# microscopic-image-analysis/DiffPointRasterisation.jl

Measured on AMD Instinct MI355X. Metric: M points/s fwd+bwd, 10M pts→256³ grid; HBM GB/s vs roofline, higher is better.
Workload: dtype f32

## Files before the change

diffpointrasterisation.jl_amd/csrc/dpr_tiled.hip:

```cpp
#include <hip/hip_runtime.h>

#include <cstring>
#include <mutex>
#include <set>
#include <type_traits>
#include <utility>

#include "dpr_tiled_impl.h"

namespace dpr {

template <int NO>
__device__ __forceinline__ int primary_tile(const int (&ref0)[NO], const TileGeom<NO>& tg) {
    int t = 0, stride = 1;
    bool in = true;
#pragma unroll
    for (int d = 0; d < NO; ++d) {
        const int r = ref0[d] < 0 ? 0 : ref0[d];
        int c = r / TileDims<NO>::T[d];
        if (d == NO - 1) {
            c -= tg.tz0;
            in = (unsigned)c < (unsigned)tg.nt[d];
        }
        t += c * stride;
// ... 422 lines not shown
                it.part_nparts = part | (k << 16);
                items[atomicAdd(&bstart[bucket], 1u)] = it;
            }
            if (k > 1) {
                slab_run += k;
                split_list[atomicAdd(&s_nsplit, 1u)] = (uint32_t)i;
            }
            run += c;
        }
    }
    if (threadIdx.x == 1023) tile_start[NT] = wbase + incl;
    __syncthreads();
    if (threadIdx.x == 0) *n_split = s_nsplit;
}

constexpr int kScanTiles = 32, kScanGroups = 1024 / kScanTiles;
__global__ __launch_bounds__(1024) void k_colscan(uint32_t* __restrict__ counts, int nblk, int NT,
                                                  uint32_t* __restrict__ totals,
                                                  uint32_t* __restrict__ zero_word = nullptr) {
    if (zero_word && blockIdx.x == 0 && threadIdx.x < 2) zero_word[threadIdx.x] = 0u;
    constexpr int kRowBatch = 16;
    __shared__ uint32_t part[kScanGroups][kScanTiles];
    const int j = threadIdx.x % kScanTiles, g = threadIdx.x / kScanTiles;
    const int tile = blockIdx.x * kScanTiles + j;
    const int rows = (nblk + kScanGroups - 1) / kScanGroups;
    const int r0 = g * rows, r1 = (r0 + rows < nblk) ? r0 + rows : nblk;
    const bool one = rows <= kRowBatch;
    const bool live = tile < NT;
    uint32_t v[kRowBatch];
    uint32_t s = 0;
    for (int rb = r0; rb < r1; rb += kRowBatch) {
#pragma unroll
        for (int k = 0; k < kRowBatch; ++k)
            v[k] = (live && rb + k < r1) ? counts[(size_t)(rb + k) * NT + tile] : 0u;
#pragma unroll
        for (int k = 0; k < kRowBatch; ++k) s += v[k];
    }
    part[g][j] = s;
    __syncthreads();
    uint32_t base = 0, total = 0;
#pragma unroll
    for (int k = 0; k < kScanGroups; ++k) {
        const uint32_t pv = part[k][j];
        if (k < g) base += pv;
        total += pv;
    }
    if (!live) return;
    for (int rb = r0; rb < r1; rb += kRowBatch) {
        if (!one) {
#pragma unroll
            for (int k = 0; k < kRowBatch; ++k)
                v[k] = (rb + k < r1) ? counts[(size_t)(rb + k) * NT + tile] : 0u;
        }
#pragma unroll
        for (int k = 0; k < kRowBatch; ++k) {
            if (rb + k < r1) counts[(size_t)(rb + k) * NT + tile] = base;
            base += v[k];
        }
    }
    if (g == 0) totals[tile] = total;
}

__global__ __launch_bounds__(1024) void k_tilescan(TileScanArgs ts) {
    tilescan_body(ts.totals, ts.NT, ts.cap, ts.tile_start, ts.items, ts.n_items, ts.tile_parts,
                  ts.tile_slab, ts.split_list, ts.n_split, ts.hdr, ts.hdr_out, ts.rot,
                  ts.rot_words, ts.trans, ts.trans_words, ts.nonzero_bins, ts.nblk);
}

}
#include "dpr_coarse.h"
namespace dpr {

template <typename T, int NI, int NO, bool HAS_PW, bool WANT_IDX>
__global__ __launch_bounds__(kBinThreads) void k_scatter(
    GridDesc<NO> gd, TileGeom<NO> tg, int64_t P, int64_t chunk, const T* __restrict__ points,
    const T* __restrict__ pw, const T* __restrict__ rot, const T* __restrict__ trans, int64_t b,
    const uint32_t* __restrict__ prefix, const uint32_t* __restrict__ tile_start,
    Rec4<T>* __restrict__ rec, uint32_t* __restrict__ rec_idx, uint32_t* __restrict__ slot_of,
    T* __restrict__ ds_dpoints, T* __restrict__ ds_dpw, int zero_dropped,
    uint32_t* __restrict__ maxpw) {
    extern __shared__ uint32_t cursor[];
    const unsigned slice = xcd_slice(blockIdx.x, gridDim.x);
    const uint32_t* row = prefix + (size_t)slice * tg.NT;
    for (int i = threadIdx.x; i < tg.NT; i += kBinThreads) cursor[i] = tile_start[i] + row[i];
    __syncthreads();
    const Pose<T, NI, NO> ps = load_pose<T, NI, NO>(rot, trans, nullptr, b);
    const int64_t lo = (int64_t)slice * chunk;
    const int64_t hi = (lo + chunk < P) ? lo + chunk : P;
    if (lo >= hi) return;
    uint32_t wkey = 0;
    int64_t p = lo + threadIdx.x;
    T nxt[NI], nxt_w = T(1);
    {
        const int64_t pl = p < hi ? p : hi - 1;
        load_point<T, NI>(points, pl, nxt);
        if (HAS_PW) nxt_w = pw[pl];
    }
#pragma unroll
    for (int j = 0; j < NI; ++j) pin_value(nxt[j]);
    if (HAS_PW) pin_value(nxt_w);
    drain_vmem();
    while (p < hi) {
        T pt[NI];
#pragma unroll
        for (int j = 0; j < NI; ++j) pt[j] = nxt[j];
        const T w = nxt_w;
        const int64_t pc = p;
        p += kBinThreads;
        {
            const int64_t pl = p < hi ? p : hi - 1;
            load_point<T, NI>(points, pl, nxt);
            if (HAS_PW) nxt_w = pw[pl];
        }
        int ref0[NO];
        T dlo[NO];
        bool valid = ref_and_deltas<T, NI, NO>(pt, ps, gd, ref0, dlo);
        const int tl = valid ? primary_tile<NO>(ref0, tg) : -1;
        valid = tl >= 0;
        uint32_t pos = (uint32_t)P;
        if (valid) pos = atomicAdd(&cursor[tl], 1u);
        if (HAS_PW && valid) wkey = wrange_merge(wkey, abs_key(w));
        Rec4<T> r;
#pragma unroll
        for (int j = 0; j < 3; ++j) r.v[j] = (j < NI) ? pt[(j < NI) ? j : 0] : T(0);
        r.v[3] = HAS_PW ? w : idx_to_slot((uint32_t)pc, T(0));
        rec[pos] = r;
        if (HAS_PW && WANT_IDX) rec_idx[pos] = (uint32_t)pc;
        if (WANT_IDX) slot_of[pc] = pos;
        if (zero_dropped && !valid) {
#pragma unroll
            for (int j = 0; j < NI; ++j) ds_dpoints[pc * NI + j] = T(0);
            if (ds_dpw) ds_dpw[pc] = T(0);
        }
    }
    if (HAS_PW) publish_max_abs(maxpw, wkey);
}

template <typename T, int NI, int NO, bool HAS_PW, int S, bool GROUP, bool W3, bool RUNS>
__device__ __forceinline__ void scatter_wc_body(
    const GridDesc<NO>& gd, const TileGeom<NO>& tg, int64_t P, int64_t chunk, const T* __restrict__ points,
    const T* __restrict__ pw, const T* __restrict__ rot, const T* __restrict__ trans, int64_t b0,
    int nb, const uint32_t* __restrict__ prefix, const uint32_t* __restrict__ tile_start,
    RecT<T, W3>* __restrict__ rec, uint32_t* __restrict__ slot_of, uint16_t* __restrict__ run_lp,
    T* __restrict__ ds_dpoints, T* __restrict__ ds_dpw, int zero_dropped, uint32_t* __restrict__ maxpw,
    int fused_scan, const TileScanArgs& ts) {
    const unsigned n_slices = fused_scan ? gridDim.x - 1u : gridDim.x;
    if (fused_scan && blockIdx.x == n_slices) {
        tilescan_body(ts.totals, ts.NT, ts.cap, ts.tile_start, ts.items, ts.n_items, ts.tile_parts,
                      ts.tile_slab, ts.split_list, ts.n_split, ts.hdr, ts.hdr_out, ts.rot,
                      ts.rot_words, ts.trans, ts.trans_words, ts.nonzero_bins, ts.nblk);
        return;
    }
    static_assert(!(W3 && HAS_PW), "compact records carry no point weight");
    static_assert(!RUNS || (!GROUP && !W3 && S <= 65536), "the sorted map: one pose, 4-word records, uint16 owners");
    constexpr int PPT = S / kWcThreads;
    uint32_t wkey = 0;
    if (!GROUP) nb = 1;
    const int NT = tg.NT, NTe = NT * nb;
    const uint32_t Pe = (uint32_t)(P * nb);
    extern __shared__ uint32_t dyn[];
    uint32_t* cursor = dyn;
    uint32_t* lhist = dyn + NTe;
    __shared__ RecT<T, W3> recs[S];
    __shared__ uint32_t dest[S];
    __shared__ uint16_t lpos[RUNS ? S : 1];
    uint32_t* const wsum = dest;
    static_assert(S >= kWcThreads / kWave, "wave sums fit");
    const unsigned slice = xcd_slice(blockIdx.x, n_slices);
    const uint32_t* row = prefix + (size_t)slice * NTe;
    constexpr int kMaxBpt = 4096 / kWcThreads;
    const int lane = threadIdx.x & (kWave - 1), wave = threadIdx.x / kWave;
    if (fused_scan) {
        const int bpe = (NTe + kWcThreads - 1) / kWcThreads;
        const int e0 = threadIdx.x * bpe;
        uint32_t c[kMaxBpt], rw[kMaxBpt], sum = 0;
#pragma unroll
        for (int q = 0; q < kMaxBpt; ++q) {
            const int i = e0 + q;
            const bool in = q < bpe && i < NTe;
            c[q] = in ? ts.totals[i] : 0u;
            rw[q] = in ? row[i] : 0u;
            sum += c[q];
        }
        uint32_t incl = sum;
#pragma unroll
        for (int o = 1; o < kWave; o <<= 1) {
            const uint32_t v = __shfl_up(incl, o, kWave);
            if (lane >= o) incl += v;
        }
        if (lane == kWave - 1) wsum[wave] = incl;
        __syncthreads();
        uint32_t run = incl - sum;
        for (int wv = 0; wv < wave; ++wv) run += wsum[wv];
#pragma unroll
        for (int q = 0; q < kMaxBpt; ++q) {
            const int i = e0 + q;
            if (q < bpe && i < NTe) cursor[i] = run + rw[q];
            run += c[q];
        }
    } else {
        for (int i = threadIdx.x; i < NTe; i += kWcThreads) cursor[i] = tile_start[i] + row[i];
    }
    for (int i = threadIdx.x; i < NT; i += kWcThreads) lhist[i] = 0;
    __syncthreads();
    const int64_t lo = (int64_t)slice * chunk;
    const int64_t hi = (lo + chunk < P) ? lo + chunk : P;
    const int bpt = (NT + kWcThreads - 1) / kWcThreads;
    const int bin0 = threadIdx.x * bpt;
    if (lo >= hi) return;
    constexpr bool kPrefetch = !GROUP;
    auto load_sub = [&](int64_t sbase, T (&dp)[PPT][NI], T (&dw)[PPT]) {
        const int64_t left = hi - sbase;
        const uint32_t n = left >= S ? (uint32_t)S : (left > 0 ? (uint32_t)left : 0u);
        const T* const pb = points + (n ? sbase : hi - 1) * NI;
        const T* const wb = HAS_PW ? pw + (n ? sbase : hi - 1) : nullptr;
#pragma unroll
        for (int k = 0; k < PPT; ++k) {
            const uint32_t lp = threadIdx.x + (uint32_t)k * kWcThreads;
            const uint32_t ll = n ? (lp < n ? lp : n - 1) : 0u;
            load_point<T, NI>(pb, (int64_t)ll, dp[k]);
            dw[k] = HAS_PW ? wb[ll] : T(1);
        }
    };
    T nxt_pt[kPrefetch ? PPT : 1][NI], nxt_w[kPrefetch ? PPT : 1];
    if constexpr (kPrefetch) load_sub(lo, nxt_pt, nxt_w);
    for (int64_t base = lo; base < hi; base += S) {
        const uint32_t nloc = (uint32_t)((hi - base < S) ? hi - base : S);
        T pt[PPT][NI], w[PPT];
        if constexpr (kPrefetch) {
#pragma unroll
            for (int k = 0; k < PPT; ++k) {
#pragma unroll
                for (int j = 0; j < NI; ++j) pt[k][j] = nxt_pt[k][j];
                w[k] = nxt_w[k];
            }
            load_sub(base + S, nxt_pt, nxt_w);
        } else {
            load_sub(base, pt, w);
        }
        for (int jp = 0; jp < (GROUP ? nb : 1); ++jp) {
            const Pose<T, NI, NO> ps = load_pose<T, NI, NO>(rot, trans, nullptr, b0 + jp);
            uint32_t* cur = cursor + jp * NT;
            uint32_t* const slot_b = slot_of ? slot_of + (size_t)jp * P + base : (uint32_t*)nullptr;
            int tile[PPT];
            uint32_t lrank[PPT];
#pragma unroll
            for (int k = 0; k < PPT; ++k) {
                const uint32_t lp = threadIdx.x + (uint32_t)k * kWcThreads;
                int ref0[NO];
                T dlo[NO];
                bool valid = ref_and_deltas<T, NI, NO>(pt[k], ps, gd, ref0, dlo) && lp < nloc;
                tile[k] = valid ? primary_tile<NO>(ref0, tg) : -1;
                valid = tile[k] >= 0;
                lrank[k] = 0;
                if (valid) lrank[k] = atomicAdd(&lhist[tile[k]], 1u);
                if (HAS_PW && valid) wkey = wrange_merge(wkey, abs_key(w[k]));
            }
            lds_barrier();
            uint32_t cnt_sum = 0;
            uint32_t cnt[kMaxBpt];
#pragma unroll
            for (int q = 0; q < kMaxBpt; ++q) {
                const int i = bin0 + q;
                cnt[q] = (q < bpt && i < NT) ? lhist[i] : 0u;
                cnt_sum += cnt[q];
            }
            uint32_t incl = cnt_sum;
#pragma unroll
            for (int o = 1; o < kWave; o <<= 1) {
                const uint32_t v = __shfl_up(incl, o, kWave);
                if (lane >= o) incl += v;
            }
            if (lane == kWave - 1) wsum[wave] = incl;
            lds_barrier();
            uint32_t run = incl - cnt_sum;
            for (int wv = 0; wv < wave; ++wv) run += wsum[wv];
            uint32_t n_valid = 0;
#pragma unroll
            for (int wv = 0; wv < kWcThreads / kWave; ++wv) n_valid += wsum[wv];
#pragma unroll
            for (int q = 0; q < kMaxBpt; ++q) {
                const int i = bin0 + q;
                if (q < bpt && i < NT) lhist[i] = run;
                run += cnt[q];
            }
            lds_barrier();
#pragma unroll
            for (int k = 0; k < PPT; ++k) {
                const uint32_t lp = threadIdx.x + (uint32_t)k * kWcThreads;
                if (tile[k] >= 0) {
                    const uint32_t sidx = lhist[tile[k]] + lrank[k];
                    const uint32_t d = cur[tile[k]] + lrank[k];
                    RecT<T, W3> r;
#pragma unroll
                    for (int j = 0; j < 3; ++j) r.v[j] = (j < NI) ? pt[k][(j < NI) ? j : 0] : T(0);
                    if constexpr (!W3) r.v[3] = HAS_PW ? w[k] : idx_to_slot((uint32_t)base + lp, T(0));
                    recs[sidx] = r;
                    dest[sidx] = d;
                    if constexpr (RUNS) lpos[sidx] = (uint16_t)lp;
                    else if (slot_b) __builtin_nontemporal_store(d, &slot_b[lp]);
                } else if (lp < nloc) {
                    if (!RUNS && slot_b) __builtin_nontemporal_store(Pe, &slot_b[lp]);
                    if (zero_dropped) {
                        T* const dp_b = ds_dpoints + base * NI;
#pragma unroll
                        for (int j = 0; j < NI; ++j) dp_b[lp * NI + j] = T(0);
                        if (ds_dpw) (ds_dpw + base)[lp] = T(0);
                    }
                }
            }
            lds_barrier();
            if constexpr (RUNS) {
                uint16_t* const lp_b = run_lp + base;
                for (uint32_t i = threadIdx.x; i < nloc; i += kWcThreads) {
                    const bool owned = i < n_valid;
                    const uint32_t d = dest[i];
                    if (owned) {
                        rec[d] = recs[i];
                        __builtin_nontemporal_store(lpos[i], &lp_b[i]);
                    }
                    __builtin_nontemporal_store(owned ? d : kRunEnd, &slot_b[i]);
                }
            } else {
                for (uint32_t i = threadIdx.x; i < n_valid; i += kWcThreads) rec[dest[i]] = recs[i];
            }
#pragma unroll
            for (int q = 0; q < kMaxBpt; ++q) {
                const int i = bin0 + q;
                if (q < bpt && i < NT) {
                    cur[i] += cnt[q];
                    lhist[i] = 0;
                }
            }
            lds_barrier();
        }
    }
    if (HAS_PW) publish_max_abs(maxpw, wkey);
}
template <typename T, int NI, int NO, bool HAS_PW, int S, bool GROUP, bool W3>
__global__ __launch_bounds__(kWcThreads) void k_scatter_wc(
    GridDesc<NO> gd, TileGeom<NO> tg, int64_t P, int64_t chunk, const T* __restrict__ points,
    const T* __restrict__ pw, const T* __restrict__ rot, const T* __restrict__ trans, int64_t b0,
    int nb, const uint32_t* __restrict__ prefix, const uint32_t* __restrict__ tile_start,
    RecT<T, W3>* __restrict__ rec, uint32_t* __restrict__ slot_of, T* __restrict__ ds_dpoints,
    T* __restrict__ ds_dpw, int zero_dropped, uint32_t* __restrict__ maxpw, int fused_scan,
    TileScanArgs ts) {
    scatter_wc_body<T, NI, NO, HAS_PW, S, GROUP, W3, false>(gd, tg, P, chunk, points, pw, rot, trans, b0, nb, prefix,
                                                            tile_start, rec, slot_of, nullptr, ds_dpoints, ds_dpw,
                                                            zero_dropped, maxpw, fused_scan, ts);
}
template <typename T, int NI, int NO, bool HAS_PW, int S>
__global__ __launch_bounds__(kWcThreads) void k_scatter_wc_runs(
    GridDesc<NO> gd, TileGeom<NO> tg, int64_t P, int64_t chunk, const T* __restrict__ points,
    const T* __restrict__ pw, const T* __restrict__ rot, const T* __restrict__ trans, int64_t b0,
    const uint32_t* __restrict__ prefix, const uint32_t* __restrict__ tile_start, Rec4<T>* __restrict__ rec,
    uint32_t* __restrict__ run_slot, uint16_t* __restrict__ run_lp, uint32_t* __restrict__ maxpw, int fused_scan,
    TileScanArgs ts) {
    scatter_wc_body<T, NI, NO, HAS_PW, S, false, false, true>(gd, tg, P, chunk, points, pw, rot, trans, b0, 1, prefix,
                                                              tile_start, rec, run_slot, run_lp, nullptr, nullptr, 0,
                                                              maxpw, fused_scan, ts);
}

struct LocalBinArgs {
    char* ws;
    size_t pose_stride;
    size_t off_rec, off_slot, off_desc, off_bdesc, off_ltot;
};
constexpr int kTouchCap = 1024;
template <typename T, int NI, int NO, bool HAS_PW, int S, bool W3, bool ONE, int TH, bool STAGE>
__global__ __launch_bounds__(TH, ((sizeof(T) == 4 && ONE) ? 8 : 4)) void k_bin_local(
    GridDesc<NO> gd, TileGeom<NO> tg, int64_t P, const T* __restrict__ points,
    const T* __restrict__ pw, const T* __restrict__ rot, const T* __restrict__ trans, int64_t b0,
    int nb, LocalBinArgs la, int want_slot, uint32_t spare_slot, T* __restrict__ ds_dpoints,
    T* __restrict__ ds_dpw, int zero_dropped) {
    static_assert(!(W3 && HAS_PW), "compact records carry no point weight");
    constexpr int PPT = S / TH;
    if (ONE) nb = 1;
    const int NT = tg.NT;
    extern __shared__ uint32_t lhist[];
    __shared__ RecT<T, W3> recs[STAGE ? S : 1];
    __shared__ uint16_t touched[kTouchCap];
    __shared__ uint32_t wsum[TH / kWave];
    __shared__ uint32_t s_ntouch, s_nvalid;
    for (int i = threadIdx.x; i < NT; i += TH) lhist[i] = 0;
    if (threadIdx.x == 0) s_ntouch = 0;
    const int64_t base = (int64_t)blockIdx.x * S;
    const uint32_t nloc = (uint32_t)((P - base < S) ? P - base : S);
    const T* const pts_blk = points + base * NI;
    const T* const pw_blk = HAS_PW ? pw + base : nullptr;
    T pt[PPT][NI], w[PPT];
#pragma unroll
    for (int k = 0; k < PPT; ++k) {
        const uint32_t lp = threadIdx.x + (uint32_t)k * TH;
        const uint32_t ll = lp < nloc ? lp : nloc - 1;
        if (nloc) {
            load_point<T, NI>(pts_blk, (int64_t)ll, pt[k]);
            w[k] = HAS_PW ? pw_blk[ll] : T(1);
        } else {
#pragma unroll
            for (int j = 0; j < NI; ++j) pt[k][j] = T(0);
            w[k] = T(1);
        }
    }
    if constexpr (HAS_PW) {
        uint32_t wkey = 0;
#pragma unroll
        for (int k = 0; k < PPT; ++k)
            if (threadIdx.x + (uint32_t)k * TH < nloc) wkey = wrange_merge(wkey, abs_key(w[k]));
        publish_max_abs((uint32_t*)(la.ws + la.off_ltot) + 2 * NT, wkey);
    }
    __syncthreads();
    const int lane = threadIdx.x & (kWave - 1), wave = threadIdx.x / kWave;
#pragma unroll 1
    for (int jp = 0; jp < nb; ++jp) {
        const Pose<T, NI, NO> ps = load_pose<T, NI, NO>(rot, trans, nullptr, b0 + jp);
        char* const wsp = la.ws + (size_t)jp * la.pose_stride;
        RecT<T, W3>* const rec_blk = (RecT<T, W3>*)(wsp + la.off_rec) + base;
        uint32_t* const slot_blk = want_slot ? (uint32_t*)(wsp + la.off_slot) + base : (uint32_t*)nullptr;
        RunDesc* const desc = (RunDesc*)(wsp + la.off_desc) + (size_t)blockIdx.x * S;
        uint32_t* const ltot = (uint32_t*)(wsp + la.off_ltot);
        int tile[PPT];
        uint32_t lrank[PPT];
        uint32_t left = 0;
#pragma unroll
        for (int k = 0; k < PPT; ++k) {
            const uint32_t lp = threadIdx.x + (uint32_t)k * TH;
            int ref0[NO];
            T dlo[NO];
            bool valid = ref_and_deltas<T, NI, NO>(pt[k], ps, gd, ref0, dlo) && lp < nloc;
            tile[k] = valid ? primary_tile<NO>(ref0, tg) : -1;
            valid = tile[k] >= 0;
            lrank[k] = 0;
            unsigned long long todo = __ballot(valid);
            int rounds = 0;
            while (todo && rounds < 8) {
                const int leader = __ffsll((long long)todo) - 1;
                const int t = __shfl(tile[k], leader, kWave);
                const unsigned long long same = __ballot(tile[k] == t) & todo;
                if (__popcll(same) < 4) break;
                uint32_t r0 = 0;
                if (lane == leader) {
                    r0 = atomicAdd(&lhist[t], (uint32_t)__popcll(same));
                    if (r0 == 0) {
                        const uint32_t pos = atomicAdd(&s_ntouch, 1u);
                        if (pos < (uint32_t)kTouchCap) touched[pos] = (uint16_t)t;
                    }
                }
                r0 = __shfl(r0, leader, kWave);
                if ((same >> lane) & 1ull) lrank[k] = r0 + (uint32_t)__popcll(same & ((1ull << lane) - 1ull));
                todo &= ~same;
                ++rounds;
            }
            if ((todo >> lane) & 1ull) left |= 1u << k;
        }
        if (__ballot(left != 0)) {
#pragma unroll
            for (int k = 0; k < PPT; ++k)
                if ((left >> k) & 1u) lrank[k] = atomicAdd(&lhist[tile[k]], 1u);
#pragma unroll
            for (int k = 0; k < PPT; ++k) {
                if (((left >> k) & 1u) && lrank[k] == 0) {
                    const uint32_t pos = atomicAdd(&s_ntouch, 1u);
                    if (pos < (uint32_t)kTouchCap) touched[pos] = (uint16_t)tile[k];
                }
            }
        }
        lds_barrier();
        const uint32_t n_t = s_ntouch;
        const bool listed = n_t <= (uint32_t)kTouchCap;
        if (listed) {
            if (wave == 0) {
                uint32_t carry = 0;
                for (uint32_t i0 = 0; i0 < n_t; i0 += kWave) {
                    const uint32_t i = i0 + lane;
// ... 1546 lines not shown
        }
    }
    const int lane = threadIdx.x & (kWave - 1), wave = threadIdx.x / kWave;
#pragma unroll
    for (int k = 0; k < NVAL; ++k) {
        const double v = (k < NVAL - 2) ? (double)vals[k < NVAL - 2 ? k : 0]
                                        : (k == NVAL - 2 ? bg_sum : sq_sum);
        const double s = wave_sum<double>(v);
        if (lane == 0) red[wave][k] = s;
    }
    __syncthreads();
    if (threadIdx.x < (rs.target ? NVAL : NVAL - 1)) {
        double s = 0.0;
#pragma unroll
        for (int w = 0; w < NW; ++w) s += red[w][threadIdx.x];
        partials[(size_t)threadIdx.x * max_items + blockIdx.x] = s;
    }
}

template <typename T> struct PoseReduceArgs {
    const double* partials;
    const WorkItem* items;
    const uint32_t* n_items;
    int max_items, NT, n_in, n_out;
    int64_t b0;
    T* ds_drotation;
    T* ds_dtranslation;
    T* ds_dbackground;
    T* ds_dout_weight;
    T* loss;
    BinHeader* hdr;
    int accumulate;
};
template <typename T>
__device__ __forceinline__ void pose_reduce_body(int k, uint32_t j, bool grouped,
                                                 const PoseReduceArgs<T>& a) {
    __shared__ double wsum[16];
    const int64_t b = a.b0 + j;
    double s = 0.0;
    const bool stale = a.hdr && a.hdr->verdict != 1u;
    if (a.hdr && k == 0 && j == 0 && threadIdx.x == 0) a.hdr->state = 0u;
    const int n = stale ? 0 : (int)*a.n_items;
    if (!grouped) {
        for (int t = threadIdx.x; t < n; t += 1024) s += a.partials[(size_t)k * a.max_items + t];
    } else {
        for (int t = threadIdx.x; t < n; t += 1024)
            if (a.items[t].tile / (uint32_t)a.NT == j) s += a.partials[(size_t)k * a.max_items + t];
    }
    s = wave_sum<double>(s);
    if ((threadIdx.x & 63) == 0) wsum[threadIdx.x >> 6] = s;
    __syncthreads();
    if (threadIdx.x == 0) {
        double tot = 0.0;
#pragma unroll
        for (int w = 0; w < 16; ++w) tot += wsum[w];
        if (stale) tot = __builtin_nan("");
        const int nr = a.n_out * a.n_in;
        T* dst = nullptr;
        if (k < nr)
            dst = &a.ds_drotation[b * nr + k];
        else if (k < nr + a.n_out)
            dst = &a.ds_dtranslation[b * a.n_out + (k - nr)];
        else if (k == nr + a.n_out)
            dst = &a.ds_dout_weight[b];
        else if (k == nr + a.n_out + 1)
            dst = &a.ds_dbackground[b];
        else if (a.loss)
            dst = &a.loss[b];
        if (dst) *dst = a.accumulate ? (T)((double)*dst + tot) : (T)tot;
    }
}

template <typename T, int NI, bool FIRST_POSE, int kUPB>
__global__ __launch_bounds__(1024) void k_unpermute(int64_t P, int nb,
                                                    const Rec4<T>* __restrict__ grad,
                                                    const uint32_t* __restrict__ slot_of,
                                                    T* __restrict__ ds_dpoints,
                                                    T* __restrict__ ds_dpw,
                                                    const BinHeader* __restrict__ hdr,
                                                    int reduce_blocks, PoseReduceArgs<T> pr,
                                                    size_t pose_stride) {
    if ((int)blockIdx.x < reduce_blocks) {
        pose_reduce_body<T>((int)blockIdx.x, 0u, false, pr);
        return;
    }
    const unsigned ublock = blockIdx.x - (unsigned)reduce_blocks;
    const unsigned ublocks = gridDim.x - (unsigned)reduce_blocks;
    bool stale = hdr && hdr->verdict != 1u;
    if (hdr && pose_stride)
        for (int j = 1; j < nb; ++j)
            stale = stale || ((const BinHeader*)((const char*)hdr + (size_t)j * pose_stride))->verdict != 1u;
    if (stale) {
        const T nan = T(__builtin_nanf(""));
        const int64_t b0 = (int64_t)ublock * (kUPB * 1024) + threadIdx.x;
#pragma unroll
        for (int k = 0; k < kUPB; ++k) {
            const int64_t p = b0 + k * 1024;
            if (p >= P) continue;
#pragma unroll
            for (int j = 0; j < NI; ++j) ds_dpoints[p * NI + j] = nan;
            if (ds_dpw) ds_dpw[p] = nan;
        }
        return;
    }
    const int64_t base = (int64_t)xcd_slice(ublock, ublocks) * (kUPB * 1024) + threadIdx.x;
    uint32_t slot[kUPB];
#pragma unroll
    for (int k = 0; k < kUPB; ++k) {
        const int64_t p = base + k * 1024;
        slot[k] = __builtin_nontemporal_load(&slot_of[p < P ? p : P - 1]);
    }
    Rec4<T> g[kUPB];
#pragma unroll
    for (int k = 0; k < kUPB; ++k) g[k] = grad[slot[k]];
    for (int j = 1; j < nb; ++j) {
        const Rec4<T>* gradj =
            pose_stride ? (const Rec4<T>*)((const char*)grad + (size_t)j * pose_stride) : grad;
        const uint32_t* slotj = pose_stride
                                    ? (const uint32_t*)((const char*)slot_of + (size_t)j * pose_stride)
                                    : slot_of + (size_t)j * P;
#pragma unroll
        for (int k = 0; k < kUPB; ++k) {
            const int64_t p = base + k * 1024;
            const Rec4<T> gj = gradj[slotj[p < P ? p : P - 1]];
#pragma unroll
            for (int c = 0; c < 4; ++c) g[k].v[c] += gj.v[c];
        }
    }
#pragma unroll
    for (int k = 0; k < kUPB; ++k) {
        const int64_t p = base + k * 1024;
        if (p >= P) continue;
        if (FIRST_POSE) {
#pragma unroll
            for (int j = 0; j < NI; ++j) __builtin_nontemporal_store(g[k].v[j], &ds_dpoints[p * NI + j]);
            if (ds_dpw) __builtin_nontemporal_store(g[k].v[3], &ds_dpw[p]);
        } else {
#pragma unroll
            for (int j = 0; j < NI; ++j) ds_dpoints[p * NI + j] += g[k].v[j];
            if (ds_dpw) ds_dpw[p] += g[k].v[3];
        }
    }
}

template <typename T, int NI, bool FIRST_POSE>
__global__ __launch_bounds__(1024, 8) void k_unpermute_runs(int64_t P, const Rec4<T>* __restrict__ grad,
                                                            const uint32_t* __restrict__ run_slot,
                                                            const uint16_t* __restrict__ run_lp,
                                                            T* __restrict__ ds_dpoints, T* __restrict__ ds_dpw,
                                                            const BinHeader* __restrict__ hdr,
                                                            int reduce_blocks, PoseReduceArgs<T> pr) {
    constexpr int S = sizeof(T) == 4 ? kWcPpt * kWcThreads : kWcPpt * kWcThreads / 2;
    constexpr int PPT = S / 1024;
    __shared__ Rec4<T> stage[S];
    if ((int)blockIdx.x < reduce_blocks) {
        pose_reduce_body<T>((int)blockIdx.x, 0u, false, pr);
        return;
    }
    const unsigned ublock = blockIdx.x - (unsigned)reduce_blocks;
    const unsigned ublocks = gridDim.x - (unsigned)reduce_blocks;
    if (hdr && hdr->verdict != 1u) {
        const T nan = T(__builtin_nanf(""));
        const int64_t b0 = (int64_t)ublock * S + threadIdx.x;
#pragma unroll
        for (int k = 0; k < PPT; ++k) {
            const int64_t p = b0 + k * 1024;
            if (p >= P) continue;
#pragma unroll
            for (int j = 0; j < NI; ++j) ds_dpoints[p * NI + j] = nan;
            if (ds_dpw) ds_dpw[p] = nan;
        }
        return;
    }
    const int64_t base = (int64_t)xcd_slice(ublock, ublocks) * S;
    const uint32_t nloc = (uint32_t)((P - base < S) ? P - base : S);
    uint32_t slot[PPT], lp[PPT];
#pragma unroll
    for (int k = 0; k < PPT; ++k) {
        const uint32_t i = threadIdx.x + (uint32_t)k * 1024;
        const uint32_t ic = i < nloc ? i : nloc - 1;
        slot[k] = __builtin_nontemporal_load(&run_slot[base + ic]);
        lp[k] = __builtin_nontemporal_load(&run_lp[base + ic]);
        if (i >= nloc) slot[k] = kRunEnd;
    }
    Rec4<T> zero;
#pragma unroll
    for (int c = 0; c < 4; ++c) zero.v[c] = T(0);
#pragma unroll
    for (int k = 0; k < PPT; ++k) stage[threadIdx.x + k * 1024] = zero;
    Rec4<T> g[PPT];
#pragma unroll
    for (int k = 0; k < PPT; ++k) {
        g[k] = zero;
        if (slot[k] < (uint64_t)P) g[k] = grad[slot[k]];
    }
    __syncthreads();
#pragma unroll
    for (int k = 0; k < PPT; ++k)
        if (slot[k] < (uint64_t)P) stage[lp[k] & (uint32_t)(S - 1)] = g[k];
    __syncthreads();
    const T* const words = &stage[0].v[0];
    T* const dp = ds_dpoints + base * NI;
    for (uint32_t e = threadIdx.x; e < nloc * NI; e += 1024) {
        const T v = words[(e / NI) * 4 + e % NI];
        if (FIRST_POSE) __builtin_nontemporal_store(v, &dp[e]);
        else dp[e] += v;
    }
    if (ds_dpw) {
        T* const dw = ds_dpw + base;
        for (uint32_t q = threadIdx.x; q < nloc; q += 1024) {
            const T v = stage[q].v[3];
            if (FIRST_POSE) __builtin_nontemporal_store(v, &dw[q]);
            else dw[q] += v;
        }
    }
}

template <typename T>
__global__ __launch_bounds__(1024) void k_pose_reduce(PoseReduceArgs<T> pr) {
    pose_reduce_body<T>((int)blockIdx.x, blockIdx.y, gridDim.y > 1, pr);
}

template <typename T, int NI>
__global__ __launch_bounds__(256) void k_unsort(int64_t P, const uint32_t* __restrict__ inv_perm,
                                                const T* __restrict__ dp_sorted,
                                                const T* __restrict__ dpw_sorted,
                                                T* __restrict__ ds_dpoints, T* __restrict__ ds_dpw,
                                                const BinHeader* __restrict__ hdr) {
    constexpr int PER = 4;
    const int64_t q0 = (int64_t)blockIdx.x * (256 * PER) + threadIdx.x;
    if (hdr && hdr->verdict != 1u) {
        const T nan = T(__builtin_nanf(""));
#pragma unroll
        for (int k = 0; k < PER; ++k) {
            const int64_t q = q0 + k * 256;
            if (q >= P) continue;
#pragma unroll
            for (int j = 0; j < NI; ++j) ds_dpoints[q * NI + j] = nan;
            if (ds_dpw) ds_dpw[q] = nan;
        }
        return;
    }
    size_t i[PER];
#pragma unroll
    for (int k = 0; k < PER; ++k) {
        const int64_t q = q0 + k * 256;
        const size_t v = inv_perm[q < P ? q : P - 1];
        i[k] = v < (size_t)P ? v : 0;
    }
    T v[PER][NI], w[PER];
#pragma unroll
    for (int k = 0; k < PER; ++k) {
#pragma unroll
        for (int j = 0; j < NI; ++j) v[k][j] = dp_sorted[i[k] * NI + j];
        w[k] = ds_dpw ? dpw_sorted[i[k]] : T(0);
    }
#pragma unroll
    for (int k = 0; k < PER; ++k) {
        const int64_t q = q0 + k * 256;
        if (q >= P) continue;
#pragma unroll
        for (int j = 0; j < NI; ++j) ds_dpoints[q * NI + j] = v[k][j];
        if (ds_dpw) ds_dpw[q] = w[k];
    }
}

static int cu_count() {
    static std::mutex mu;
    static int cus[64] = {0};
    int dev = 0;
    if (hipGetDevice(&dev) != hipSuccess || dev < 0 || dev >= 64) return 256;
    std::lock_guard<std::mutex> lock(mu);
    if (!cus[dev]) {
        int n = 0;
        if (hipDeviceGetAttribute(&n, hipDeviceAttributeMultiprocessorCount, dev) != hipSuccess || n < 1) n = 256;
        cus[dev] = n;
    }
    return cus[dev];
}

struct PoseWs {
    char* base;
    const Plan& pl;
    template <typename X> X* at(size_t off) const { return (X*)(base + off); }
    BinHeader* hdr() const { return at<BinHeader>(pl.off_hdr); }
    uint32_t* counts() const { return at<uint32_t>(pl.off_counts); }
    uint32_t* totals() const { return at<uint32_t>(pl.off_totals); }
    uint32_t* tile_start() const { return at<uint32_t>(pl.off_tile_start); }
    WorkItem* items() const { return at<WorkItem>(pl.off_items); }
    uint32_t* n_items() const { return at<uint32_t>(pl.off_nitems); }
    uint32_t* weight_keys() const { return n_items() + 2; }
    uint32_t* nzbins() const { return at<uint32_t>(pl.off_nzbins); }
    uint32_t* tparts() const { return at<uint32_t>(pl.off_tparts); }
    uint32_t* tslab() const { return at<uint32_t>(pl.off_tslab); }
    uint32_t* n_split() const { return at<uint32_t>(pl.off_split); }
    uint32_t* split() const { return n_split() + 1; }
    template <typename R> R* rec() const { return at<R>(pl.off_rec); }
    uint32_t* idx() const { return at<uint32_t>(pl.off_idx); }
    uint32_t* slot() const { return at<uint32_t>(pl.off_slot); }
    RunDesc* sdesc() const { return at<RunDesc>(pl.off_sdesc); }
    uint32_t* ltot() const { return at<uint32_t>(pl.off_ltot); }
    uint32_t max_rec() const { return (uint32_t)(pl.nsub * pl.sub); }
};

struct PoseWalk {
    const Plan& pl;
    char* ws;
    bool kept;
    int64_t B;
    int64_t group(int64_t b) const {
        int64_t nb = 1;
        while (nb * 2 <= pl.bg && b + nb * 2 <= B) nb *= 2;
        return nb;
    }
    int64_t copy_of(int64_t b) const { return kept && B > 1 ? b : (pl.local ? b % pl.lb : 0); }
    PoseWs at(int64_t b) const { return {ws + (size_t)copy_of(b) * pl.pose_stride, pl}; }
    bool opens_local_batch(int64_t b) const { return b % pl.lb == 0; }
    int local_batch(int64_t b) const { return (int)((B - b < pl.lb) ? B - b : pl.lb); }
};

template <typename K> static int allow_dynamic_lds(K kernel, size_t bytes, int max_bytes) {
    if (bytes <= 48 * 1024) return DPR_OK;
    static std::mutex mu;
    static std::set<std::pair<const void*, int>> done;
    int dev = 0;
    DPR_HIP(hipGetDevice(&dev));
    std::lock_guard<std::mutex> lock(mu);
    if (done.count({(const void*)kernel, dev})) return DPR_OK;
    DPR_HIP(hipFuncSetAttribute((const void*)kernel, hipFuncAttributeMaxDynamicSharedMemorySize, max_bytes));
    done.insert({(const void*)kernel, dev});
    return DPR_OK;
}


static bool scatter_is_wc(int NT, int nb) { return NT * nb <= 4096; }

static bool records_are_compact(int NT, int nb, bool has_pw, bool want_idx) {
    return !has_pw && !want_idx && scatter_is_wc(NT, nb);
}

template <typename T, int NI, int NO, bool HAS_PW, bool WANT_IDX>
static int launch_scatter(hipStream_t st, const GridDesc<NO>& gd, const TileGeom<NO>& tg,
                          const Plan& pl, const PoseWs& w, int64_t P, const T* points, const T* pw,
                          const T* rot, const T* trans, int64_t b, int nb, const TileScanArgs& ts,
                          bool fused) {
    if (scatter_is_wc(tg.NT, nb)) {
        constexpr int S = (sizeof(T) == 4) ? kWcPpt * kWcThreads : kWcPpt * kWcThreads / 2;
        const size_t lds2 = (size_t)tg.NT * (nb + 1) * 4;
#define DPR_LAUNCH_WC(GROUP, W3)                                                                  \
    hipLaunchKernelGGL((k_scatter_wc<T, NI, NO, HAS_PW, S, GROUP, W3>),                          \
                       dim3(pl.nblk + (fused ? 1 : 0)),                                          \
                       dim3(kWcThreads), lds2, st, gd, tg, P, pl.chunk, points, pw, rot, trans, \
// ... 627 lines not shown
```

diffpointrasterisation.jl_amd/csrc/dpr_tiled_impl.h:

```cpp
#pragma once
#include <hip/hip_runtime.h>

#include "../../include/dpr.h"
#include "dpr_device.h"
#include "dpr_jvp.h"
#include "dpr_tiled.h"

namespace dpr {

template <int NO> struct TileDims;
template <> struct TileDims<3> {
    static constexpr int T[3] = {64, 16, 8};
};
template <> struct TileDims<2> {
    static constexpr int T[3] = {32, 32, 1};
};
constexpr int kMaxTiles = 32768;
constexpr int kBinThreads = 1024;
constexpr int kWcThreads = 1024;
constexpr int kWcPpt = 4;
constexpr int kSplatThreads = 512;
constexpr int kSplatRunsOcc = 4;
template <typename T> __host__ __device__ constexpr int gather_threads() {
    return sizeof(T) == 8 ? 512 : 256;
}
template <typename T> __host__ __device__ constexpr int gather_waves_per_simd() { return 4; }
constexpr int kUpb = 4;
constexpr int kGatherRb = 8;
constexpr int kMaxBinBlocks = 512;
constexpr int kSplitChunks = 8;
constexpr int kSplitRows = 16;
constexpr int kSplitGrid = 2048;

template <int NO> struct TileGeom {
    int nt[NO];
    int NT;
    int tz0;
    int ghost;
};

template <int NO> __host__ __device__ constexpr int tile_voxels() {
    int v = 1;
    for (int d = 0; d < NO; ++d) v *= TileDims<NO>::T[d];
    return v;
}
template <int NO> __host__ __device__ constexpr int tile_voxels_halo() {
    int v = 1;
    for (int d = 0; d < NO; ++d) v *= TileDims<NO>::T[d] + 1;
    return v;
}
template <int NO> __host__ __device__ constexpr int halo_count() {
    return tile_voxels_halo<NO>() - tile_voxels<NO>();
}

struct SlabCut {
    int per_layer, layers, lps, nslab;
};

constexpr uint32_t kBinMagic = 0x44505242u, kBinValid = 1u;
struct alignas(16) BinHeader {
    uint32_t magic, state;
    uint32_t elem, n_in, n_out, has_pw;
    int64_t P;
    int32_t grid[3];
    uint32_t verdict;
    uint64_t points, pw;
    uint32_t layout, pad_[3];
    unsigned char pose[96];
};

struct alignas(16) WorkItem {
    uint32_t tile, begin, end;
    uint32_t part_nparts;
};

struct alignas(8) RunDesc {
    uint32_t start;
    uint32_t tile_count;
    __host__ __device__ uint32_t tile() const { return tile_count & 0x7fffu; }
    __host__ __device__ uint32_t count() const { return tile_count >> 15; }
};
constexpr int kMaxLocalTiles = 16384;
constexpr int kMaxRuns = 256;
constexpr int kMaxRunsGather = 64;

constexpr uint32_t kRunEnd = 0xffffffffu;
struct Plan {
    int bg;
    int nblk;
    int64_t chunk;
    uint32_t cap;
    int max_items;
    int max_slabs;
    bool run_map;
    size_t off_hdr, off_counts, off_totals, off_tile_start, off_items, off_nitems, off_nzbins, off_tparts, off_tslab,
        off_split, off_rec, off_idx, off_slot, off_aux, total;
    bool sort_inside;
    size_t off_spts, off_spw, off_perm, off_iperm, off_sgrad, off_sgradw, off_sorttmp;
    size_t pose_stride;
    bool local;
    int lb;
    int64_t copies;
    int sub;
    int64_t nsub;
    int64_t max_desc;
    size_t off_ltot, off_dstart, off_dcursor, off_bdesc, off_desc, off_sdesc;
};

template <int NO> bool make_slab_cut(const int64_t* grid, SlabCut* sc);
template <int NO> TileGeom<NO> slab_geom(const int64_t* grid, const SlabCut& sc, int s, bool forward);
int slab_max_tiles(const SlabCut& sc);

struct PlanRequest {
    size_t elem;
    int n_in, n_out;
    int tiles;
    int64_t P, B;
    int max_group;
    bool coherent;
    bool share_batch;
    bool slabbed;
    bool fwd_only;
};
PlanRequest plan_request(size_t elem, int op, unsigned flags, int n_in, int n_out, const SlabCut& sc, int64_t P,
                         int64_t B);
Plan make_plan(const PlanRequest& rq);
Plan pose_plan(size_t elem, int n_in, int n_out, const SlabCut& sc, int64_t P);
uint32_t plan_layout_id(const Plan& pl);
int tiled_check(int n_out, const int64_t* grid, int64_t P, unsigned flags, const char* binning_flag, SlabCut* sc);
bool pose_binning_cut(int n_out, const int64_t* grid, int64_t P, SlabCut* sc);
size_t channel_part_bytes(size_t elem, int64_t P, int C);
size_t jvp_part_bytes(size_t elem, int64_t P);

size_t coarse_workspace_bytes(size_t elem, int64_t P);

}
```

diffpointrasterisation.jl_amd/csrc/dpr_tiled_plan.hip:

```cpp
#include <cstdlib>

#include "dpr_tiled_impl.h"

namespace dpr {

static int max_tiles() {
    static const int v = [] {
        const char* e = getenv("DPR_MAX_TILES");
        int x = e ? atoi(e) : kMaxTiles;
        return x < 16 ? 16 : (x > kMaxTiles ? kMaxTiles : x);
    }();
    return v;
}
template <int NO> bool make_slab_cut(const int64_t* grid, SlabCut* sc) {
    const int cap = max_tiles();
    int64_t per = 1;
    for (int d = 0; d + 1 < NO; ++d) per *= (grid[d] + TileDims<NO>::T[d] - 1) / TileDims<NO>::T[d];
    const int64_t layers = (grid[NO - 1] + TileDims<NO>::T[NO - 1] - 1) / TileDims<NO>::T[NO - 1];
    if (per > cap / 2 || layers > (1 << 20)) return false;
    sc->per_layer = (int)per;
    sc->layers = (int)layers;
    if (per * layers <= cap) {
        sc->lps = (int)layers;
        sc->nslab = 1;
// ... 47 lines not shown
    PlanRequest rq{};
    rq.elem = elem;
    rq.n_in = n_in;
    rq.n_out = n_out;
    rq.tiles = slab_max_tiles(sc);
    rq.P = P;
    rq.B = B;
    rq.max_group = max_pose_group(flags);
    rq.coherent = (flags & DPR_FLAG_COHERENT_POINTS) != 0;
    rq.share_batch = (flags & 3u) != 0;
    rq.slabbed = sc.nslab > 1;
    rq.fwd_only = op == DPR_OP_RASTER && !(flags & 3u);
    return rq;
}

Plan pose_plan(size_t elem, int n_in, int n_out, const SlabCut& sc, int64_t P) {
    return make_plan(PlanRequest{.elem = elem, .n_in = n_in, .n_out = n_out, .tiles = slab_max_tiles(sc), .P = P,
                                 .B = 1, .max_group = 1, .fwd_only = true});
}

Plan make_plan(const PlanRequest& rq) {
    const size_t elem = rq.elem;
    const int n_in = rq.n_in, n_out = rq.n_out, NT1 = rq.tiles;
    const int64_t P1 = rq.P, B = rq.B;
    const bool slabbed = rq.slabbed, fwd_only = rq.fwd_only;
    const bool coherent = rq.coherent && !slabbed;
    const bool share_batch = rq.share_batch && B > 1;
    const int max_group = share_batch ? 1 : rq.max_group;
    Plan pl;
    pl.pose_stride = 0;
    pl.sort_inside = !coherent && NT1 > 4096 && B >= 4 && P1 >= 200000;
    pl.bg = pose_group(NT1, P1, B, max_group);
    pl.local = (coherent || pl.sort_inside) && !slabbed && NT1 <= kMaxLocalTiles &&
               pl.bg == 1;
    pl.lb = 1;
    if (pl.local && B > 1) {
        if (share_batch) {
            pl.lb = B < 16 ? (int)B : 16;
        } else {
            pl.lb = B < 8 ? (int)B : 8;
            while (pl.lb > 1 && P1 * pl.lb > ((int64_t)1 << 29)) --pl.lb;
        }
    }
    pl.copies = share_batch ? B : pl.lb;
    const int NT = NT1 * pl.bg;
    const int64_t P = P1 * pl.bg;
    int64_t nblk, chunk;
    if (NT <= 4096) {
        const int64_t sub = (elem == 4) ? kWcPpt * kWcThreads : kWcPpt * kWcThreads / 2;
        chunk = ((P1 + 255) / 256 + sub - 1) / sub * sub;
        if (chunk < sub) chunk = sub;
    } else {
        nblk = (P1 + 8191) / 8192;
        if (nblk < 1) nblk = 1;
        if (nblk > kMaxBinBlocks) nblk = kMaxBinBlocks;
        chunk = (P1 + nblk - 1) / nblk;
        chunk = (chunk + kBinThreads - 1) / kBinThreads * kBinThreads;
        if (chunk < kBinThreads) chunk = kBinThreads;
    }
    nblk = (P1 + chunk - 1) / chunk;
    if (nblk < 1) nblk = 1;
    pl.nblk = (int)nblk;
    pl.chunk = chunk;
    size_t o = 0;
    auto take = [&o](size_t bytes) {
        const size_t at = o;
        o += align_up(bytes);
        return at;
    };
    pl.off_hdr = take(sizeof(BinHeader));
    pl.off_counts = take((size_t)nblk * NT * 4);
    pl.off_totals = take((size_t)NT * 4);
    pl.off_tile_start = take((size_t)(NT + 1) * 4);
    int64_t cap = P / 256;
    const int64_t cap_min = fwd_only ? 2 * 4096 : 4096;
    if (cap < cap_min) cap = cap_min;
    if (n_out == 2) {
        cap = P / 2048;
        if (cap < 2048) cap = 2048;
    }
    pl.cap = (uint32_t)cap;
    pl.max_slabs = (int)(2 * ((P + cap - 1) / cap) + 1);
    pl.max_items = NT + pl.max_slabs;
    pl.off_items = take((size_t)pl.max_items * sizeof(WorkItem));
    pl.off_nitems = take(4);
    pl.off_nzbins = take((size_t)kMaxBinBlocks * 4);
    pl.off_tparts = take((size_t)NT * 4);
    pl.off_tslab = take((size_t)NT * 4);
    pl.off_split = take((size_t)(pl.max_slabs / 2 + 2) * 4);
    pl.sub = elem == 4 ? 4096 : 2048;
    pl.run_map = pl.bg == 1 && !pl.local && NT1 <= 4096 && pl.copies == 1;
    pl.nsub = (P1 + pl.sub - 1) / pl.sub;
    if (pl.nsub < 1) pl.nsub = 1;
    pl.max_desc = 0;
    int64_t nrec = P;
    if (pl.local) {
        pl.max_desc = pl.nsub * pl.sub;
        nrec = pl.nsub * pl.sub;
        pl.off_ltot = take((size_t)(2 * NT1 + 2) * 4);
        pl.off_dcursor = take((size_t)NT1 * 4);
        pl.off_dstart = take((size_t)(NT1 + 1) * 4);
        pl.off_bdesc = take((size_t)pl.nsub * 4);
        pl.off_desc = take((size_t)pl.max_desc * sizeof(RunDesc));
        pl.off_sdesc = take((size_t)pl.max_desc * sizeof(RunDesc));
    }
    pl.off_rec = take((size_t)(nrec + 1) * 4 * elem);
    pl.off_idx = take((size_t)(P1 + 1) * 4);
    pl.off_slot = take((size_t)(P + 1) * 4);
    if (pl.copies > 1) {
        pl.pose_stride = o;
        o += (size_t)(pl.copies - 1) * pl.pose_stride;
    }
    pl.off_spts = pl.off_spw = pl.off_perm = pl.off_iperm = pl.off_sgrad = pl.off_sgradw = pl.off_sorttmp = o;
    if (pl.sort_inside) {
        pl.off_spts = take((size_t)P1 * n_in * elem);
        pl.off_spw = take((size_t)P1 * elem);
        pl.off_perm = o;
        pl.off_iperm = take((size_t)P1 * 4);
        pl.off_sgrad = take((size_t)P1 * n_in * elem);
        pl.off_sgradw = take((size_t)P1 * elem);
        pl.off_sorttmp = take(coarse_workspace_bytes(elem, P1));
    }
    pl.off_aux = o;
    const size_t nvh = (n_out == 3) ? tile_voxels_halo<3>() : tile_voxels_halo<2>();
    const size_t halo = align_up((size_t)NT * ((n_out == 3) ? halo_count<3>() : halo_count<2>()) * elem) +
                        align_up((size_t)pl.max_slabs * nvh * elem);
    const size_t partials = (size_t)pl.max_items * 16 * 8;
    o += align_up(halo > partials ? halo : partials);
    pl.total = o;
    return pl;
}

uint32_t plan_layout_id(const Plan& pl) {
    uint64_t h = 1469598103934665603ull;
    auto mix = [&](uint64_t v) {
        for (int i = 0; i < 8; ++i) {
            h ^= (v >> (8 * i)) & 0xffu;
            h *= 1099511628211ull;
        }
    };
    mix(pl.local ? 1 : 0);
    mix((uint64_t)pl.bg);
    mix((uint64_t)pl.sub);
    mix((uint64_t)pl.cap);
    mix(pl.off_items);
    mix(pl.off_rec);
    mix(pl.off_idx);
    mix(pl.off_slot);
    mix(pl.off_aux);
    mix(pl.local ? pl.off_sdesc : 0);
    mix(pl.pose_stride);
    mix(pl.off_iperm);
    mix((uint64_t)pl.lb);
    mix(pl.run_map ? 1 : 0);
    const uint32_t id = (uint32_t)(h ^ (h >> 32));
    return id ? id : 1u;
}

static bool grid_cut(int n_out, const int64_t* grid, SlabCut* sc) {
    return n_out == 3 ? make_slab_cut<3>(grid, sc) : make_slab_cut<2>(grid, sc);
}

bool tiled_supported(int n_out, const int64_t* grid) {
    SlabCut sc;
    return grid_cut(n_out, grid, &sc);
}

int tiled_slabs(int n_out, const int64_t* grid) {
    SlabCut sc;
    return grid_cut(n_out, grid, &sc) ? sc.nslab : 0;
}

bool tiled_preferred(int op, int n_out, const int64_t* grid, int64_t P, int64_t B, int64_t G) {
    (void)G;
    if (P >= (int64_t)1 << 32) return false;
    SlabCut sc;
    if (!grid_cut(n_out, grid, &sc)) return false;
    const int64_t NT_all = (int64_t)sc.per_layer * sc.layers;
    const int64_t per_tile = op == DPR_OP_RASTER ? (n_out == 3 ? 60 : 48)
                                                 : (n_out == 3 ? 320 : (NT_all <= 4096 ? 150 : 430));
    if (P < per_tile * NT_all) return false;
    if (sc.nslab > 1) {
        return op == DPR_OP_RASTER && P >= 1000000;
    }
    const int NT = sc.per_layer * sc.layers;
    const bool grouped = B >= 4 && pose_group(NT, P, B, 0) >= 4;
    if (op == DPR_OP_RASTER && B < 4 && (NT <= 64 || (n_out == 3 && NT <= 256))) return P >= 100000;
    if (op == DPR_OP_RASTER) return P >= (grouped ? 60000 : 250000);
    if (B >= 4) return P >= (grouped ? 300000 : 600000);
    return P >= 250000;
}

int tiled_tiles(int n_out, const int64_t* grid) {
    SlabCut sc;
    return grid_cut(n_out, grid, &sc) ? slab_max_tiles(sc) : -1;
}

bool tiled_batch_share_ok(int n_out, const int64_t* grid, int64_t P, int64_t B) {
    if (B < 2 || P < 1 || P * B > ((int64_t)1 << 29)) return false;
    SlabCut sc;
    if (!grid_cut(n_out, grid, &sc) || sc.nslab != 1) return false;
    return sc.per_layer * sc.layers * 2 > 4096;
}

int tiled_check(int n_out, const int64_t* grid, int64_t P, unsigned flags, const char* binning_flag, SlabCut* sc) {
    const bool quiet = !binning_flag;
    if (!grid_cut(n_out, grid, sc))
        return quiet ? DPR_ERR_UNSUPPORTED_ALGO
                     : fail(DPR_ERR_UNSUPPORTED_ALGO,
                            "DPR_ALGO_TILED: a tile layer of the grid has more than %d tiles", kMaxTiles / 2);
    if (P >= (int64_t)1 << 32)
        return quiet ? DPR_ERR_UNSUPPORTED_ALGO
                     : fail(DPR_ERR_UNSUPPORTED_ALGO, "DPR_ALGO_TILED: P must be < 2^32");
    if (sc->nslab > 1 && (flags & 3u))
        return quiet ? DPR_ERR_UNSUPPORTED_ALGO
                     : fail(DPR_ERR_UNSUPPORTED_ALGO,
                            "DPR_ALGO_TILED: a grid of more than %d tiles is processed in slabs, whose "
                            "binning cannot be kept (%s)", kMaxTiles, binning_flag);
    return DPR_OK;
}

size_t tiled_workspace_bytes(size_t elem, int op, unsigned flags, int n_in, int n_out,
                             const int64_t* grid, int64_t P, int64_t B) {
    (void)op;
    SlabCut sc;
    if (tiled_check(n_out, grid, P, flags, nullptr, &sc)) return (size_t)-1;
    return make_plan(plan_request(elem, DPR_OP_PULLBACK, flags, n_in, n_out, sc, P, B)).total;
}

bool pose_binning_cut(int n_out, const int64_t* grid, int64_t P, SlabCut* sc) {
    return tiled_check(n_out, grid, P, 0u, nullptr, sc) == DPR_OK && sc->nslab == 1;
}

bool tiled_channels_supported(int n_out, const int64_t* grid, int64_t P) {
    SlabCut sc;
    return pose_binning_cut(n_out, grid, P, &sc);
}

size_t channel_part_bytes(size_t elem, int64_t P, int C) {
    return align_up((size_t)C * (size_t)(P + 1) * elem) + align_up((size_t)C * 2 * 4);
}

size_t tiled_channels_workspace_bytes(size_t elem, int n_in, int n_out, const int64_t* grid, int64_t P,
                                      int64_t B, int C) {
    SlabCut sc;
    if (!pose_binning_cut(n_out, grid, P, &sc)) return (size_t)-1;
    size_t base = tiled_workspace_bytes(elem, DPR_OP_RASTER, 0u, n_in, n_out, grid, P, B);
    const size_t own = pose_plan(elem, n_in, n_out, sc, P).total;
    if (own > base) base = own;
    return base + channel_part_bytes(elem, P, C);
}

size_t jvp_part_bytes(size_t elem, int64_t P) {
    return align_up((size_t)(P + 1) * 4 * elem) + align_up(2 * 4);
}

size_t tiled_jvp_workspace_bytes(size_t elem, int n_in, int n_out, const int64_t* grid, int64_t P) {
    SlabCut sc;
    if (!pose_binning_cut(n_out, grid, P, &sc)) return (size_t)-1;
    return align_up(pose_plan(elem, n_in, n_out, sc, P).total) + jvp_part_bytes(elem, P);
}

}
```

Measured before the change: 28600.

## Compress sorted run map into run-start table with 12-bit owner words

Replaces the per-point 32-bit destination slot in the sorted run map with a per-segment run-start table. The slot is recovered in the unpermute kernel from a wave ballot of run-start flags plus a shuffle and a distance offset. Each 16-bit owner word now carries a run-start bit and 12 index bits, and slot stores are written only at run starts. This cuts scatter writes and is meant to make the gather reads more compact, at the cost of extra ballot, popcount and shuffle work and a limit of 4096 points per sub-block.

```diff
diff --git a/diffpointrasterisation.jl_amd/csrc/dpr_run_map.h b/diffpointrasterisation.jl_amd/csrc/dpr_run_map.h
--- /dev/null
+++ b/diffpointrasterisation.jl_amd/csrc/dpr_run_map.h
@@ -0,0 +1,95 @@
+#pragma once
+#include <stdint.h>
+
+#ifndef DPR_HD
+#if defined(__HIPCC__)
+#define DPR_HD __host__ __device__ __forceinline__
+#else
+#define DPR_HD inline
+#endif
+#endif
+
+namespace dpr {
+
+constexpr uint32_t kRunMapVersion = 2;
+constexpr int kRunMaxSub = 4096;
+constexpr int kRunSegment = 64;
+constexpr uint32_t kRunStart = 0x8000u, kRunOwnerBits = 0x0fffu, kRunSpare = 0x7000u;
+constexpr uint16_t kRunNone = 0x7fffu;
+
+DPR_HD bool run_starts(uint32_t sidx, uint32_t rank) { return rank == 0u || sidx % (uint32_t)kRunSegment == 0u; }
+DPR_HD uint16_t run_owner_word(uint32_t lp, bool first) { return (uint16_t)((lp & kRunOwnerBits) | (first ? kRunStart : 0u)); }
+DPR_HD bool run_owner_valid(uint32_t w) { return (w & kRunSpare) == 0u; }
+template <int S> DPR_HD uint32_t run_owner_index(uint32_t w) {
+    static_assert(S <= kRunMaxSub && (S & (S - 1)) == 0 && S % kRunSegment == 0, "an owner word holds 12 index bits");
+    return w & (uint32_t)(S - 1);
+}
+
+DPR_HD uint32_t run_table_index(uint32_t i, uint64_t starts, uint32_t l) {
+    return i - l + (uint32_t)__builtin_popcountll(starts & ((1ull << l) - 1ull));
+}
+DPR_HD bool run_segment_decode(uint64_t starts, uint32_t l, uint32_t& j, uint32_t& dist) {
+    const uint64_t upto = starts & (~0ull >> (63u - l));
+    j = ((uint32_t)__builtin_popcountll(upto) - 1u) & 63u;
+    dist = upto ? l - (63u - (uint32_t)__builtin_clzll(upto)) : 0u;
+    return upto != 0ull;
+}
+
+template <int S>
+uint32_t run_map_encode(const int* tile, uint32_t nloc, int NT, uint32_t* cursor, uint16_t* owner, uint32_t* table,
+                        uint32_t* dest, uint32_t* lhist , uint32_t* lrank ) {
+    static_assert(S <= kRunMaxSub, "an owner word holds 12 index bits");
+    uint32_t sorted_dest[S];
+    for (int t = 0; t < NT; ++t) lhist[t] = 0;
+    for (uint32_t lp = 0; lp < nloc; ++lp)
+        if (tile[lp] >= 0) lrank[lp] = lhist[tile[lp]]++;
+    uint32_t n_valid = 0;
+    for (int t = 0; t < NT; ++t) {
+        const uint32_t cnt = lhist[t];
+        lhist[t] = n_valid;
+        n_valid += cnt;
+    }
+    for (uint32_t lp = 0; lp < nloc; ++lp) {
+        if (tile[lp] < 0) continue;
+        const uint32_t sidx = lhist[tile[lp]] + lrank[lp];
+        owner[sidx] = run_owner_word(lp, run_starts(sidx, lrank[lp]));
+        sorted_dest[sidx] = dest[lp] = cursor[tile[lp]] + lrank[lp];
+    }
+    uint32_t runs = 0;
+    for (uint32_t seg0 = 0; seg0 < nloc; seg0 += kRunSegment) {
+        uint64_t starts = 0;
+        for (uint32_t l = 0; l < (uint32_t)kRunSegment && seg0 + l < nloc; ++l) {
+            if (seg0 + l >= n_valid) owner[seg0 + l] = kRunNone;
+            else if (owner[seg0 + l] & kRunStart) starts |= 1ull << l;
+        }
+        for (uint32_t l = 0; l < (uint32_t)kRunSegment; ++l)
+            if (starts >> l & 1u) table[run_table_index(seg0 + l, starts, l)] = sorted_dest[seg0 + l];
+        runs += (uint32_t)__builtin_popcountll(starts);
+    }
+    for (int t = 0; t < NT; ++t) {
+        const uint32_t next = t + 1 < NT ? lhist[t + 1] : n_valid;
+        cursor[t] += next - lhist[t];
+    }
+    return runs;
+}
+
+template <int S>
+void run_map_decode(const uint16_t* owner, const uint32_t* table, uint32_t nloc, uint64_t P, uint32_t* slot, uint32_t* lp,
+                    bool* has) {
+    for (uint32_t seg0 = 0; seg0 < nloc; seg0 += kRunSegment) {
+        uint64_t starts = 0;
+        for (uint32_t l = 0; l < (uint32_t)kRunSegment && seg0 + l < nloc; ++l)
+            if (owner[seg0 + l] & kRunStart) starts |= 1ull << l;
+        for (uint32_t l = 0; l < (uint32_t)kRunSegment && seg0 + l < nloc; ++l) {
+            const uint32_t i = seg0 + l;
+            uint32_t j, dist;
+            has[i] = run_segment_decode(starts, l, j, dist) && run_owner_valid(owner[i]);
+            if (!has[i]) continue;
+            slot[i] = table[seg0 + j] + dist;
+            lp[i] = run_owner_index<S>(owner[i]);
+            has[i] = slot[i] < P;
+        }
+    }
+}
+
+}
diff --git a/diffpointrasterisation.jl_amd/csrc/dpr_tiled.hip b/diffpointrasterisation.jl_amd/csrc/dpr_tiled.hip
--- a/diffpointrasterisation.jl_amd/csrc/dpr_tiled.hip
+++ b/diffpointrasterisation.jl_amd/csrc/dpr_tiled.hip
@@ -598,7 +598,7 @@
         return;
     }
     static_assert(!(W3 && HAS_PW), "compact records carry no point weight");
-    static_assert(!RUNS || (!GROUP && !W3 && S <= 65536), "the sorted map: one pose, 4-word records, uint16 owners");
+    static_assert(!RUNS || (!GROUP && !W3 && S <= kRunMaxSub), "the sorted map: one pose, 4-word records, 12-bit owners");
     constexpr int PPT = S / kWcThreads;
     uint32_t wkey = 0;
     if (!GROUP) nb = 1;
@@ -743,7 +743,7 @@
                     if constexpr (!W3) r.v[3] = HAS_PW ? w[k] : idx_to_slot((uint32_t)base + lp, T(0));
                     recs[sidx] = r;
                     dest[sidx] = d;
-                    if constexpr (RUNS) lpos[sidx] = (uint16_t)lp;
+                    if constexpr (RUNS) lpos[sidx] = run_owner_word(lp, run_starts(sidx, lrank[k]));
                     else if (slot_b) __builtin_nontemporal_store(d, &slot_b[lp]);
                 } else if (lp < nloc) {
                     if (!RUNS && slot_b) __builtin_nontemporal_store(Pe, &slot_b[lp]);
@@ -761,11 +761,12 @@
                 for (uint32_t i = threadIdx.x; i < nloc; i += kWcThreads) {
                     const bool owned = i < n_valid;
                     const uint32_t d = dest[i];
-                    if (owned) {
-                        rec[d] = recs[i];
-                        __builtin_nontemporal_store(lpos[i], &lp_b[i]);
-                    }
-                    __builtin_nontemporal_store(owned ? d : kRunEnd, &slot_b[i]);
+                    const uint32_t ow = owned ? lpos[i] : kRunNone;
+                    if (owned) rec[d] = recs[i];
+                    __builtin_nontemporal_store((uint16_t)ow, &lp_b[i]);
+                    const bool st = owned && (ow & kRunStart);
+                    const uint64_t starts = __ballot(st);
+                    if (st) __builtin_nontemporal_store(d, &slot_b[run_table_index(i, starts, (uint32_t)lane)]);
                 }
             } else {
                 for (uint32_t i = threadIdx.x; i < n_valid; i += kWcThreads) rec[dest[i]] = recs[i];
@@ -2618,6 +2619,7 @@
                                                             int reduce_blocks, PoseReduceArgs<T> pr) {
     constexpr int S = sizeof(T) == 4 ? kWcPpt * kWcThreads : kWcPpt * kWcThreads / 2;
     constexpr int PPT = S / 1024;
+    static_assert(kRunSegment == kWave && 1024 % kRunSegment == 0, "a wave holds whole segments");
     __shared__ Rec4<T> stage[S];
     if ((int)blockIdx.x < reduce_blocks) {
         pose_reduce_body<T>((int)blockIdx.x, 0u, false, pr);
@@ -2640,30 +2642,41 @@
     }
     const int64_t base = (int64_t)xcd_slice(ublock, ublocks) * S;
     const uint32_t nloc = (uint32_t)((P - base < S) ? P - base : S);
-    uint32_t slot[PPT], lp[PPT];
+    const uint32_t lane = threadIdx.x & (kWave - 1);
+    uint32_t own[PPT], tab[PPT];
 #pragma unroll
     for (int k = 0; k < PPT; ++k) {
         const uint32_t i = threadIdx.x + (uint32_t)k * 1024;
         const uint32_t ic = i < nloc ? i : nloc - 1;
-        slot[k] = __builtin_nontemporal_load(&run_slot[base + ic]);
-        lp[k] = __builtin_nontemporal_load(&run_lp[base + ic]);
-        if (i >= nloc) slot[k] = kRunEnd;
+        own[k] = __builtin_nontemporal_load(&run_lp[base + ic]);
+        if (i >= nloc) own[k] = kRunNone;
+        tab[k] = __builtin_nontemporal_load(&run_slot[base + ic]);
     }
     Rec4<T> zero;
 #pragma unroll
     for (int c = 0; c < 4; ++c) zero.v[c] = T(0);
-#pragma unroll
-    for (int k = 0; k < PPT; ++k) stage[threadIdx.x + k * 1024] = zero;
+    uint32_t slot[PPT];
+    bool has[PPT];
+#pragma unroll
+    for (int k = 0; k < PPT; ++k) {
+        const uint64_t starts = __ballot((own[k] & kRunStart) != 0u);
+        uint32_t j, dist;
+        has[k] = run_segment_decode(starts, lane, j, dist) && run_owner_valid(own[k]);
+        slot[k] = (uint32_t)__shfl((int)tab[k], (int)j, kWave) + dist;
+        has[k] = has[k] && slot[k] < (uint64_t)P;
+    }
     Rec4<T> g[PPT];
 #pragma unroll
     for (int k = 0; k < PPT; ++k) {
         g[k] = zero;
-        if (slot[k] < (uint64_t)P) g[k] = grad[slot[k]];
-    }
+        if (has[k]) g[k] = grad[slot[k]];
+    }
+#pragma unroll
+    for (int k = 0; k < PPT; ++k) stage[threadIdx.x + k * 1024] = zero;
     __syncthreads();
 #pragma unroll
     for (int k = 0; k < PPT; ++k)
-        if (slot[k] < (uint64_t)P) stage[lp[k] & (uint32_t)(S - 1)] = g[k];
+        if (has[k]) stage[run_owner_index<S>(own[k])] = g[k];
     __syncthreads();
     const T* const words = &stage[0].v[0];
     T* const dp = ds_dpoints + base * NI;
diff --git a/diffpointrasterisation.jl_amd/csrc/dpr_tiled_impl.h b/diffpointrasterisation.jl_amd/csrc/dpr_tiled_impl.h
--- a/diffpointrasterisation.jl_amd/csrc/dpr_tiled_impl.h
+++ b/diffpointrasterisation.jl_amd/csrc/dpr_tiled_impl.h
@@ -4,6 +4,7 @@
 #include "../../include/dpr.h"
 #include "dpr_device.h"
 #include "dpr_jvp.h"
+#include "dpr_run_map.h"
 #include "dpr_tiled.h"
 
 namespace dpr {
@@ -84,7 +85,6 @@
 constexpr int kMaxRuns = 256;
 constexpr int kMaxRunsGather = 64;
 
-constexpr uint32_t kRunEnd = 0xffffffffu;
 struct Plan {
     int bg;
     int nblk;
diff --git a/diffpointrasterisation.jl_amd/csrc/dpr_tiled_plan.hip b/diffpointrasterisation.jl_amd/csrc/dpr_tiled_plan.hip
--- a/diffpointrasterisation.jl_amd/csrc/dpr_tiled_plan.hip
+++ b/diffpointrasterisation.jl_amd/csrc/dpr_tiled_plan.hip
@@ -223,7 +223,7 @@
     mix(pl.pose_stride);
     mix(pl.off_iperm);
     mix((uint64_t)pl.lb);
-    mix(pl.run_map ? 1 : 0);
+    mix(pl.run_map ? kRunMapVersion : 0);
     const uint32_t id = (uint32_t)(h ^ (h >> 32));
     return id ? id : 1u;
 }
```

Result: faster. 29060 (median of 6 runs) (+1.6%).
